# godk1122/IsaacLab

Hardware: AMD Instinct MI355X
Metric: env-steps/sec (whole node), Anymal-C rough 4096 envs/GPU, RSL-RL PPO iteration (collect+GAE+update) (higher is better)
Workload: dtype f32; 1 GPU; Isaac-Velocity-Rough-Anymal-C-v0, 4096 envs/GPU, T=24, 5 epochs x 4 minibatches, terrain 1204008 triangles, 4 state snapshots resident in HBM; parallelism=dp1, rollout=hipGraph, full_step=False, update=hipGraph (measured eager 16.72 ms, graph 16.06 ms), policy_params=571801

## Files before the change

isaaclab_amd/csrc/mlp_fwd.hip:

```cpp
#include "imx_internal.h"

typedef float f32x16 __attribute__((ext_vector_type(16)));

namespace {

constexpr int FW_KMAX = 256;
constexpr int FW_ROWS = 32;
constexpr int FW_KP = FW_KMAX + 4;
constexpr int FW_COLS = 128;

__device__ __forceinline__ int acc_row32(int reg, int half) { return (reg & 3) + 8 * (reg >> 2) + 4 * half; }

template <bool ELU, bool FULL>
__device__ __forceinline__ void store_rows(const f32x16& acc, float bias, float alpha, float* y, int64_t ldy, int rows, int half) {
#pragma unroll
    for (int g = 0; g < 4; ++g) {
        float* yg = y + (int64_t)(8 * g) * ldy;
#pragma unroll
        for (int j = 0; j < 4; ++j) {
            float x = acc[4 * g + j] + bias;
            if (ELU) {
                const float e = (__expf(fminf(x, 0.0f)) - 1.0f) * alpha;
                x = x <= 0.0f ? e : x;
            }
            if (FULL || 8 * g + j + 4 * half < rows) yg[0] = x;
            yg += ldy;
        }
    }
}

__device__ __forceinline__ void store_tile(const f32x16& acc, float bias, float alpha, int elu, float* y, int64_t ldy, int rows, int half) {
    if (rows >= FW_ROWS) {
        if (elu) store_rows<true, true>(acc, bias, alpha, y, ldy, rows, half);
        else store_rows<false, true>(acc, bias, alpha, y, ldy, rows, half);
    } else {
        if (elu) store_rows<true, false>(acc, bias, alpha, y, ldy, rows, half);
        else store_rows<false, false>(acc, bias, alpha, y, ldy, rows, half);
    }
}

struct FwArgs {
    int64_t M;
    int N, K;
    const float* X;
    int64_t ldx;
    const float* W;
    const float* b;
    float* Y;
    int64_t ldy;
    float alpha;
    int ncb;
    int rs;
    int64_t rps;
    int elu;
};

template <int NS, bool XVEC>
__global__ void __launch_bounds__(256, 2) k_mlp_fwd_elu(FwArgs a) {
    static_assert(NS % 4 == 0 && 2 * NS <= FW_KMAX, "step count");
    __shared__ __attribute__((aligned(16))) float sA[2][FW_ROWS * FW_KP];
    const int t = threadIdx.x, lane = t & 63, w = t >> 6, r = lane & 31, half = lane >> 5;
    const int cb = blockIdx.x % a.ncb, split = blockIdx.x / a.ncb;
    const int col = cb * FW_COLS + w * 32 + r;
    const bool col_ok = col < a.N;
    const int K = a.K;
    float breg[NS];
    {
        const float* wr = a.W + (size_t)(col_ok ? col : a.N - 1) * K;
#pragma unroll
        for (int s = 0; s < NS; ++s) {
            const int k = half * NS + s;
            const float v = wr[k < K ? k : K - 1];
            breg[s] = (k < K && col_ok) ? v : 0.0f;
        }
    }
    const float bias = col_ok ? a.b[col] : 0.0f;
    const int64_t m_begin = (int64_t)split * a.rps, m_end = min(m_begin + a.rps, a.M);
    const int ntile = (int)((m_end - m_begin + FW_ROWS - 1) / FW_ROWS);
    constexpr int C4 = 2 * NS / 4;
    constexpr int NV = (FW_ROWS * C4 + 255) / 256;
    float4 pre[NV];
    auto g_load = [&](int tile) {
        const int64_t row0 = m_begin + (int64_t)tile * FW_ROWS;
#pragma unroll
        for (int i = 0; i < NV; ++i) {
            const int idx = t + 256 * i;
            const int rr = idx / C4, c4 = idx - rr * C4;
            const int64_t row = min(row0 + rr, m_end - 1);
            const int k0 = 4 * c4;
            const float* p = a.X + row * a.ldx + (k0 < K ? k0 : 0);
            float4 v;
            if (XVEC) {
                v = *reinterpret_cast<const float4*>(p);
            } else {
                v.x = p[0];
                v.y = p[k0 + 1 < K ? 1 : 0];
                v.z = p[k0 + 2 < K ? 2 : 0];
                v.w = p[k0 + 3 < K ? 3 : 0];
            }
            v.x = k0 + 0 < K ? v.x : 0.f;
            v.y = k0 + 1 < K ? v.y : 0.f;
            v.z = k0 + 2 < K ? v.z : 0.f;
            v.w = k0 + 3 < K ? v.w : 0.f;
            pre[i] = v;
        }
    };
    auto s_store = [&](int buf) {
#pragma unroll
        for (int i = 0; i < NV; ++i) {
            const int idx = t + 256 * i;
            const int rr = idx / C4, c4 = idx - rr * C4;
            if (FW_ROWS * C4 % 256 == 0 || rr < FW_ROWS) *reinterpret_cast<float4*>(sA[buf] + rr * FW_KP + 4 * c4) = pre[i];
        }
    };
    if (ntile > 0) {
        g_load(0);
        s_store(0);
    }
    __syncthreads();
    for (int tile = 0; tile < ntile; ++tile) {
        const int buf = tile & 1;
        if (tile + 1 < ntile) g_load(tile + 1);
        f32x16 acc;
#pragma unroll
        for (int q = 0; q < 16; ++q) acc[q] = 0.0f;
        const float4* pa = reinterpret_cast<const float4*>(sA[buf] + r * FW_KP + half * NS);
#pragma unroll
        for (int s4 = 0; s4 < NS / 4; ++s4) {
            const float4 av = pa[s4];
            acc = __builtin_amdgcn_mfma_f32_32x32x2f32(av.x, breg[4 * s4 + 0], acc, 0, 0, 0);
            acc = __builtin_amdgcn_mfma_f32_32x32x2f32(av.y, breg[4 * s4 + 1], acc, 0, 0, 0);
            acc = __builtin_amdgcn_mfma_f32_32x32x2f32(av.z, breg[4 * s4 + 2], acc, 0, 0, 0);
            acc = __builtin_amdgcn_mfma_f32_32x32x2f32(av.w, breg[4 * s4 + 3], acc, 0, 0, 0);
        }
        const int64_t row0 = m_begin + (int64_t)tile * FW_ROWS;
        if (col_ok) store_tile(acc, bias, a.alpha, a.elu, a.Y + (row0 + 4 * half) * a.ldy + col, a.ldy, (int)min<int64_t>(m_end - row0, FW_ROWS), half);
        if (tile + 1 < ntile) s_store(buf ^ 1);
        __syncthreads();
    }
}

template <int NS>
__global__ void __launch_bounds__(256, 2) k_mlp_fwd_elu_dma(FwArgs a) {
    static_assert(NS % 4 == 0 && 2 * NS <= FW_KMAX, "step count");
    __shared__ __attribute__((aligned(16))) float sA[2][FW_ROWS * FW_KP];
    const int t = threadIdx.x, lane = t & 63, w = t >> 6, r = lane & 31, half = lane >> 5;
    const int nb = gridDim.x, per = nb >> 3;
    const int vb = (nb & 7) == 0 ? (int)(blockIdx.x & 7) * per + (int)(blockIdx.x >> 3) : (int)blockIdx.x;
    const int cb = vb % a.ncb, split = vb / a.ncb;
    const int col = cb * FW_COLS + w * 32 + r;
    const bool col_ok = col < a.N;
    const int K = a.K;
    float breg[NS];
    const unsigned lds_base = (unsigned)(uintptr_t)(__attribute__((address_space(3))) float*)&sA[0][0];
    {
        float* wl = &sA[0][0] + (w & 1) * (FW_ROWS * FW_KP);
        const int64_t blk0 = (int64_t)(cb * FW_COLS + w * 32) * K;
        const int64_t avail = min<int64_t>((int64_t)32 * K, (int64_t)a.N * K - blk0);
        const bool wvec = ((reinterpret_cast<uintptr_t>(a.W) & 15) == 0);
        const float* wrow = wl + r * K + half * NS;
        for (int turn = 0; turn < 2; ++turn) {
            if ((w >> 1) == turn) {
                const int64_t avail4 = avail & ~(int64_t)3;
                if (wvec && avail4 >= 4) {
                    const unsigned wl_lds = lds_base + (unsigned)((w & 1) * FW_ROWS * FW_KP * 4);
                    for (int i = 0; i < 32 * K; i += 256) {
                        const float* src = a.W + blk0 + min<int64_t>(i + 4 * lane, avail4 - 4);
                        unsigned keep;
                        asm volatile("s_mov_b32 %0, m0\n\ts_mov_b32 m0, %2\n\ts_nop 0\n\tglobal_load_lds_dwordx4 %1, off\n\ts_mov_b32 m0, %0"
                                     : "=&s"(keep) : "v"(src), "s"(__builtin_amdgcn_readfirstlane(wl_lds + (unsigned)i * 4u)) : "memory");
                    }
                    asm volatile("s_waitcnt vmcnt(0)" ::: "memory");
                    if (lane < avail - avail4) wl[avail4 + lane] = a.W[blk0 + avail4 + lane];
                } else {
                    for (int i = 4 * lane; i < 32 * K; i += 256) {
                        float4 v = make_float4(0.f, 0.f, 0.f, 0.f);
                        const float* src = a.W + blk0 + i;
                        if (i + 4 <= avail) {
                            if (wvec) v = *reinterpret_cast<const float4*>(src);
                            else { v.x = src[0]; v.y = src[1]; v.z = src[2]; v.w = src[3]; }
                        } else {
                            if (i + 0 < avail) v.x = src[0];
                            if (i + 1 < avail) v.y = src[1];
                            if (i + 2 < avail) v.z = src[2];
                        }
                        *reinterpret_cast<float4*>(wl + i) = v;
                    }
                }
#pragma unroll
                for (int s = 0; s < NS; ++s) {
                    const int k = half * NS + s;
                    const float v = wrow[k < K ? s : 0];
                    breg[s] = (k < K && col_ok) ? v : 0.0f;
                }
            }
            __syncthreads();
        }
    }
    const float bias = col_ok ? a.b[col] : 0.0f;
    const int64_t m_begin = (int64_t)split * a.rps, m_end = min(m_begin + a.rps, a.M);
    const int ntile = (int)((m_end - m_begin + FW_ROWS - 1) / FW_ROWS);
    constexpr int C4 = 2 * NS / 4;
    const int k0 = 4 * lane;
    const int64_t lane_off = (lane < C4 && k0 < K) ? k0 : 0;
    const int nz = 2 * NS - K;
    auto dma_tile = [&](int tile, int buf) {
        const int64_t row0 = m_begin + (int64_t)tile * FW_ROWS + 8 * w;
#pragma unroll
        for (int i = 0; i < 8; ++i) {
            const int64_t row = min(row0 + i, m_end - 1);
            const float* src = a.X + row * a.ldx + lane_off;
            const unsigned dst = lds_base + (unsigned)((buf * FW_ROWS + 8 * w + i) * FW_KP * 4);
            unsigned keep;
            asm volatile("s_mov_b32 %0, m0\n\ts_mov_b32 m0, %2\n\ts_nop 0\n\tglobal_load_lds_dwordx4 %1, off\n\ts_mov_b32 m0, %0"
                         : "=&s"(keep) : "v"(src), "s"(__builtin_amdgcn_readfirstlane(dst)) : "memory");
        }
    };
    const int zoff = lane < 8 * nz ? (8 * w + lane / nz) * FW_KP + K + lane % nz : -1;
    auto zero_tail = [&](int buf) {
        if (zoff >= 0) sA[buf][zoff] = 0.0f;
        for (int i = lane + 64; i < 8 * nz; i += 64) {
            const int rr = i / nz, c = i - rr * nz;
            sA[buf][(8 * w + rr) * FW_KP + K + c] = 0.0f;
        }
    };
    if (ntile > 0) {
        dma_tile(0, 0);
        asm volatile("s_waitcnt vmcnt(0)" ::: "memory");
        zero_tail(0);
    }
    __syncthreads();
    auto mfma_tile = [&](int buf, f32x16& acc) {
        const float4* pa = reinterpret_cast<const float4*>(sA[buf] + r * FW_KP + half * NS);
#pragma unroll
        for (int s4 = 0; s4 < NS / 4; ++s4) {
            const float4 av = pa[s4];
            acc = __builtin_amdgcn_mfma_f32_32x32x2f32(av.x, breg[4 * s4 + 0], acc, 0, 0, 0);
            acc = __builtin_amdgcn_mfma_f32_32x32x2f32(av.y, breg[4 * s4 + 1], acc, 0, 0, 0);
            acc = __builtin_amdgcn_mfma_f32_32x32x2f32(av.z, breg[4 * s4 + 2], acc, 0, 0, 0);
            acc = __builtin_amdgcn_mfma_f32_32x32x2f32(av.w, breg[4 * s4 + 3], acc, 0, 0, 0);
        }
    };
    auto end_of_tile = [&](int tile, bool stores_behind) {
        if (stores_behind) asm volatile("s_waitcnt vmcnt(16)" ::: "memory");
        else asm volatile("s_waitcnt vmcnt(0)" ::: "memory");
        if (tile + 1 < ntile) zero_tail((tile & 1) ^ 1);
        asm volatile("s_waitcnt lgkmcnt(0)" ::: "memory");
        __builtin_amdgcn_s_barrier();
    };
    const bool pipelined = a.elu && (cb + 1) * FW_COLS <= a.N && ntile >= 2;
    if (pipelined) {
        f32x16 prev;
#pragma unroll
        for (int q = 0; q < 16; ++q) prev[q] = 0.0f;
        dma_tile(1, 1);
        mfma_tile(0, prev);
        end_of_tile(0, false);
        for (int tile = 1; tile < ntile; ++tile) {
            const int buf = tile & 1;
            if (tile + 1 < ntile) dma_tile(tile + 1, buf ^ 1);
            f32x16 acc;
#pragma unroll
            for (int q = 0; q < 16; ++q) acc[q] = 0.0f;
            float* y = a.Y + (m_begin + (int64_t)(tile - 1) * FW_ROWS + 4 * half) * a.ldy + col;
            const float4* pa = reinterpret_cast<const float4*>(sA[buf] + r * FW_KP + half * NS);
            constexpr int EVERY = (NS / 4) / 16 >= 1 ? (NS / 4) / 16 : 1;
#pragma unroll
            for (int s4 = 0; s4 < NS / 4; ++s4) {
                const float4 av = pa[s4];
                acc = __builtin_amdgcn_mfma_f32_32x32x2f32(av.x, breg[4 * s4 + 0], acc, 0, 0, 0);
                acc = __builtin_amdgcn_mfma_f32_32x32x2f32(av.y, breg[4 * s4 + 1], acc, 0, 0, 0);
                acc = __builtin_amdgcn_mfma_f32_32x32x2f32(av.z, breg[4 * s4 + 2], acc, 0, 0, 0);
                acc = __builtin_amdgcn_mfma_f32_32x32x2f32(av.w, breg[4 * s4 + 3], acc, 0, 0, 0);
                if (s4 % EVERY == 0 && s4 / EVERY < 16) {
                    const int q = s4 / EVERY;
                    float x = prev[q] + bias;
                    const float e = (__expf(fminf(x, 0.0f)) - 1.0f) * a.alpha;
                    x = x <= 0.0f ? e : x;
                    *y = x;
                    y += ((q & 3) == 3 ? 5 : 1) * a.ldy;
                    __builtin_amdgcn_sched_barrier(0);
                }
            }
            static_assert(NS / 4 >= 16, "sixteen output rows need sixteen blocks");
            end_of_tile(tile, true);
            prev = acc;
        }
        const int64_t row0 = m_begin + (int64_t)(ntile - 1) * FW_ROWS;
        store_tile(prev, bias, a.alpha, a.elu, a.Y + (row0 + 4 * half) * a.ldy + col, a.ldy, (int)min<int64_t>(m_end - row0, FW_ROWS), half);
        return;
    }
    for (int tile = 0; tile < ntile; ++tile) {
        const int buf = tile & 1;
        if (tile + 1 < ntile) dma_tile(tile + 1, buf ^ 1);
        f32x16 acc;
#pragma unroll
        for (int q = 0; q < 16; ++q) acc[q] = 0.0f;
        mfma_tile(buf, acc);
        const int64_t row0 = m_begin + (int64_t)tile * FW_ROWS;
        asm volatile("s_waitcnt vmcnt(0)" ::: "memory");
        if (tile + 1 < ntile) zero_tail(buf ^ 1);
        if (col_ok) store_tile(acc, bias, a.alpha, a.elu, a.Y + (row0 + 4 * half) * a.ldy + col, a.ldy, (int)min<int64_t>(m_end - row0, FW_ROWS), half);
        asm volatile("s_waitcnt lgkmcnt(0)" ::: "memory");
        __builtin_amdgcn_s_barrier();
    }
}

template <bool XVEC>
void launch_fwd(const FwArgs& a, dim3 grid, hipStream_t st) {
    const dim3 block(256);
    const int ns = (a.K + 1) / 2;
    if (ns <= 32) hipLaunchKernelGGL((k_mlp_fwd_elu<32, XVEC>), grid, block, 0, st, a);
    else if (ns <= 64) hipLaunchKernelGGL((k_mlp_fwd_elu<64, XVEC>), grid, block, 0, st, a);
    else if (XVEC && ns <= 96) hipLaunchKernelGGL((k_mlp_fwd_elu_dma<96>), grid, block, 0, st, a);
    else if (XVEC && ns <= 120) hipLaunchKernelGGL((k_mlp_fwd_elu_dma<120>), grid, block, 0, st, a);
    else if (XVEC) hipLaunchKernelGGL((k_mlp_fwd_elu_dma<128>), grid, block, 0, st, a);
    else if (ns <= 96) hipLaunchKernelGGL((k_mlp_fwd_elu<96, false>), grid, block, 0, st, a);
    else if (ns <= 120) hipLaunchKernelGGL((k_mlp_fwd_elu<120, false>), grid, block, 0, st, a);
    else hipLaunchKernelGGL((k_mlp_fwd_elu<128, false>), grid, block, 0, st, a);
}

}

extern "C" int imx_mlp_fwd_elu(int64_t M, int N, int K, const float* X_d, int64_t ldx, const float* W_d, const float* b_d, float elu_alpha,
                               int apply_elu, float* Y_d, int64_t ldy, imx_stream_t stream) {
    IMX_REQUIRE(M > 0 && N > 0 && K > 0 && X_d && W_d && b_d && Y_d, "imx_mlp_fwd_elu: bad arguments");
    IMX_REQUIRE(K <= FW_KMAX, "imx_mlp_fwd_elu: %d in-features (at most %d: the weights of a column live in registers)", K, FW_KMAX);
    IMX_REQUIRE(ldx >= K && ldy >= N, "imx_mlp_fwd_elu: row pitch smaller than the row");
    static int num_cu = 0;
    if (num_cu == 0) {
        int dev = 0;
        if (hipGetDevice(&dev) != hipSuccess || hipDeviceGetAttribute(&num_cu, hipDeviceAttributeMultiprocessorCount, dev) != hipSuccess || num_cu <= 0)
            num_cu = 256;
    }
    FwArgs a;
    a.M = M; a.N = N; a.K = K; a.X = X_d; a.ldx = ldx; a.W = W_d; a.b = b_d; a.Y = Y_d; a.ldy = ldy; a.alpha = elu_alpha; a.elu = apply_elu;
    a.ncb = (N + FW_COLS - 1) / FW_COLS;
    int64_t rs = std::max<int64_t>(1, (2 * (int64_t)num_cu) / a.ncb);
    rs = std::min<int64_t>(rs, std::max<int64_t>(1, M / (4 * FW_ROWS)));
    a.rps = ((M + rs - 1) / rs + FW_ROWS - 1) / FW_ROWS * FW_ROWS;
    a.rs = (int)((M + a.rps - 1) / a.rps);
    const bool xvec = (ldx % 4 == 0) && ((reinterpret_cast<uintptr_t>(X_d) & 15) == 0) && (K % 4 == 0 || ldx >= ((K + 3) & ~3));
    const dim3 grid((unsigned)(a.ncb * a.rs));
    if (xvec) launch_fwd<true>(a, grid, (hipStream_t)stream);
    else launch_fwd<false>(a, grid, (hipStream_t)stream);
    IMX_HIP(hipGetLastError());
    return 0;
}
```

Before: 5.283 million env-steps/s.

## Split MLP forward into MFMA waves and helper waves for DMA and epilogue

Replaces the 256-thread DMA forward kernel for wide inputs (K>128) with a 512-thread warp-specialized kernel. Four waves run only MFMA and stage raw accumulators into LDS. Four helper waves prefetch X tiles with global_load_lds, then apply bias and ELU and write vectorized rows one tile behind. The weight block is loaded cooperatively by all waves in one pass, and the grid is sized for one workgroup per CU. This is meant to hide store and activation latency behind matrix math, at the cost of extra LDS traffic, lower occupancy and an extra barrier per tile.

```diff
diff --git a/isaaclab_amd/csrc/mlp_fwd.hip b/isaaclab_amd/csrc/mlp_fwd.hip
--- a/isaaclab_amd/csrc/mlp_fwd.hip
+++ b/isaaclab_amd/csrc/mlp_fwd.hip
@@ -1,6 +1,7 @@
 #include "imx_internal.h"
 
 typedef float f32x16 __attribute__((ext_vector_type(16)));
+typedef float f32x4 __attribute__((ext_vector_type(4)));
 
 namespace {
 
@@ -140,64 +141,36 @@
     }
 }
 
+constexpr int FW_SP = FW_COLS + 4;
+
 template <int NS>
-__global__ void __launch_bounds__(256, 2) k_mlp_fwd_elu_dma(FwArgs a) {
-    static_assert(NS % 4 == 0 && 2 * NS <= FW_KMAX, "step count");
-    __shared__ __attribute__((aligned(16))) float sA[2][FW_ROWS * FW_KP];
+struct FwLds {
+    static constexpr int TILE = FW_ROWS * FW_KP;
+    static constexpr int STAGE = FW_ROWS * FW_SP;
+    static constexpr int WBLK = FW_COLS * 2 * NS;
+    static constexpr bool T0_FREE = (TILE + WBLK) * 4 <= 160 * 1024;
+    static constexpr int W_OFF = T0_FREE ? TILE : 0;
+    static constexpr int LOOP = 2 * TILE + 2 * STAGE;
+    static constexpr int TOTAL = W_OFF + WBLK > LOOP ? W_OFF + WBLK : LOOP;
+};
+
+template <int NS>
+__global__ void __launch_bounds__(512, 1) k_mlp_fwd_elu_roles(FwArgs a) {
+    static_assert(NS % 8 == 0 && 2 * NS <= FW_KMAX, "step count");
+    using L = FwLds<NS>;
+    static_assert(L::TOTAL * 4 <= 160 * 1024, "LDS");
+    __shared__ __attribute__((aligned(16))) float lds[L::TOTAL];
+    float* const sA = lds;
+    float* const sS = lds + 2 * L::TILE;
+    float* const wl = lds + L::W_OFF;
     const int t = threadIdx.x, lane = t & 63, w = t >> 6, r = lane & 31, half = lane >> 5;
+    const bool helper = w >= 4;
+    const int h = w & 3;
     const int nb = gridDim.x, per = nb >> 3;
     const int vb = (nb & 7) == 0 ? (int)(blockIdx.x & 7) * per + (int)(blockIdx.x >> 3) : (int)blockIdx.x;
     const int cb = vb % a.ncb, split = vb / a.ncb;
-    const int col = cb * FW_COLS + w * 32 + r;
-    const bool col_ok = col < a.N;
     const int K = a.K;
-    float breg[NS];
-    const unsigned lds_base = (unsigned)(uintptr_t)(__attribute__((address_space(3))) float*)&sA[0][0];
-    {
-        float* wl = &sA[0][0] + (w & 1) * (FW_ROWS * FW_KP);
-        const int64_t blk0 = (int64_t)(cb * FW_COLS + w * 32) * K;
-        const int64_t avail = min<int64_t>((int64_t)32 * K, (int64_t)a.N * K - blk0);
-        const bool wvec = ((reinterpret_cast<uintptr_t>(a.W) & 15) == 0);
-        const float* wrow = wl + r * K + half * NS;
-        for (int turn = 0; turn < 2; ++turn) {
-            if ((w >> 1) == turn) {
-                const int64_t avail4 = avail & ~(int64_t)3;
-                if (wvec && avail4 >= 4) {
-                    const unsigned wl_lds = lds_base + (unsigned)((w & 1) * FW_ROWS * FW_KP * 4);
-                    for (int i = 0; i < 32 * K; i += 256) {
-                        const float* src = a.W + blk0 + min<int64_t>(i + 4 * lane, avail4 - 4);
-                        unsigned keep;
-                        asm volatile("s_mov_b32 %0, m0\n\ts_mov_b32 m0, %2\n\ts_nop 0\n\tglobal_load_lds_dwordx4 %1, off\n\ts_mov_b32 m0, %0"
-                                     : "=&s"(keep) : "v"(src), "s"(__builtin_amdgcn_readfirstlane(wl_lds + (unsigned)i * 4u)) : "memory");
-                    }
-                    asm volatile("s_waitcnt vmcnt(0)" ::: "memory");
-                    if (lane < avail - avail4) wl[avail4 + lane] = a.W[blk0 + avail4 + lane];
-                } else {
-                    for (int i = 4 * lane; i < 32 * K; i += 256) {
-                        float4 v = make_float4(0.f, 0.f, 0.f, 0.f);
-                        const float* src = a.W + blk0 + i;
-                        if (i + 4 <= avail) {
-                            if (wvec) v = *reinterpret_cast<const float4*>(src);
-                            else { v.x = src[0]; v.y = src[1]; v.z = src[2]; v.w = src[3]; }
-                        } else {
-                            if (i + 0 < avail) v.x = src[0];
-                            if (i + 1 < avail) v.y = src[1];
-                            if (i + 2 < avail) v.z = src[2];
-                        }
-                        *reinterpret_cast<float4*>(wl + i) = v;
-                    }
-                }
-#pragma unroll
-                for (int s = 0; s < NS; ++s) {
-                    const int k = half * NS + s;
-                    const float v = wrow[k < K ? s : 0];
-                    breg[s] = (k < K && col_ok) ? v : 0.0f;
-                }
-            }
-            __syncthreads();
-        }
-    }
-    const float bias = col_ok ? a.b[col] : 0.0f;
+    const unsigned lds_base = (unsigned)(uintptr_t)(__attribute__((address_space(3))) float*)&lds[0];
     const int64_t m_begin = (int64_t)split * a.rps, m_end = min(m_begin + a.rps, a.M);
     const int ntile = (int)((m_end - m_begin + FW_ROWS - 1) / FW_ROWS);
     constexpr int C4 = 2 * NS / 4;
@@ -205,116 +178,178 @@
     const int64_t lane_off = (lane < C4 && k0 < K) ? k0 : 0;
     const int nz = 2 * NS - K;
     auto dma_tile = [&](int tile, int buf) {
-        const int64_t row0 = m_begin + (int64_t)tile * FW_ROWS + 8 * w;
+        const int64_t row0 = m_begin + (int64_t)tile * FW_ROWS + 8 * h;
 #pragma unroll
         for (int i = 0; i < 8; ++i) {
             const int64_t row = min(row0 + i, m_end - 1);
             const float* src = a.X + row * a.ldx + lane_off;
-            const unsigned dst = lds_base + (unsigned)((buf * FW_ROWS + 8 * w + i) * FW_KP * 4);
+            const unsigned dst = lds_base + (unsigned)((buf * FW_ROWS + 8 * h + i) * FW_KP * 4);
             unsigned keep;
             asm volatile("s_mov_b32 %0, m0\n\ts_mov_b32 m0, %2\n\ts_nop 0\n\tglobal_load_lds_dwordx4 %1, off\n\ts_mov_b32 m0, %0"
                          : "=&s"(keep) : "v"(src), "s"(__builtin_amdgcn_readfirstlane(dst)) : "memory");
         }
     };
-    const int zoff = lane < 8 * nz ? (8 * w + lane / nz) * FW_KP + K + lane % nz : -1;
+    const int zoff = lane < 8 * nz ? (8 * h + lane / nz) * FW_KP + K + lane % nz : -1;
     auto zero_tail = [&](int buf) {
-        if (zoff >= 0) sA[buf][zoff] = 0.0f;
+        float* tb = sA + buf * L::TILE;
+        if (zoff >= 0) tb[zoff] = 0.0f;
         for (int i = lane + 64; i < 8 * nz; i += 64) {
             const int rr = i / nz, c = i - rr * nz;
-            sA[buf][(8 * w + rr) * FW_KP + K + c] = 0.0f;
-        }
-    };
-    if (ntile > 0) {
-        dma_tile(0, 0);
+            tb[(8 * h + rr) * FW_KP + K + c] = 0.0f;
+        }
+    };
+    {
+        const int64_t cb0 = (int64_t)cb * FW_COLS * K;
+        const int64_t avail = min<int64_t>((int64_t)FW_COLS * K, (int64_t)a.N * K - cb0);
+        const int64_t avail4 = avail & ~(int64_t)3;
+        const bool wdma = ((reinterpret_cast<uintptr_t>(a.W) & 15) == 0) && avail4 >= 4;
+        if (wdma) {
+            for (int i = 256 * w; i < FW_COLS * K; i += 8 * 256) {
+                const float* src = a.W + cb0 + min<int64_t>(i + 4 * lane, avail4 - 4);
+                unsigned keep;
+                asm volatile("s_mov_b32 %0, m0\n\ts_mov_b32 m0, %2\n\ts_nop 0\n\tglobal_load_lds_dwordx4 %1, off\n\ts_mov_b32 m0, %0"
+                             : "=&s"(keep) : "v"(src), "s"(__builtin_amdgcn_readfirstlane(lds_base + (unsigned)(L::W_OFF + i) * 4u)) : "memory");
+            }
+        } else {
+            for (int i = 4 * t; i < FW_COLS * K; i += 4 * 512) {
+                float4 v = make_float4(0.f, 0.f, 0.f, 0.f);
+                const float* src = a.W + cb0 + i;
+                if (i + 0 < avail) v.x = src[0];
+                if (i + 1 < avail) v.y = src[1];
+                if (i + 2 < avail) v.z = src[2];
+                if (i + 3 < avail) v.w = src[3];
+                *reinterpret_cast<float4*>(wl + i) = v;
+            }
+        }
+        if (L::T0_FREE && helper && ntile > 0) dma_tile(0, 0);
         asm volatile("s_waitcnt vmcnt(0)" ::: "memory");
-        zero_tail(0);
+        if (L::T0_FREE && helper && ntile > 0) zero_tail(0);
+        __syncthreads();
+        if (wdma && t < avail - avail4) wl[avail4 + t] = a.W[cb0 + avail4 + t];
+        __syncthreads();
+    }
+    if (!helper) {
+        const int col = cb * FW_COLS + w * 32 + r;
+        const bool col_ok = col < a.N;
+        float breg[NS];
+        {
+            const float* wrow = wl + (w * 32 + r) * K + half * NS;
+#pragma unroll
+            for (int s = 0; s < NS; ++s) {
+                const int k = half * NS + s;
+                const float v = wrow[k < K ? s : 0];
+                breg[s] = (k < K && col_ok) ? v : 0.0f;
+            }
+        }
+        asm volatile("s_waitcnt lgkmcnt(0)" ::: "memory");
+        if (!L::T0_FREE) __syncthreads();
+        __syncthreads();
+        for (int tile = 0; tile < ntile; ++tile) {
+            const int buf = tile & 1;
+            f32x16 acc;
+#pragma unroll
+            for (int q = 0; q < 16; ++q) acc[q] = 0.0f;
+            const float4* pa = reinterpret_cast<const float4*>(sA + buf * L::TILE + r * FW_KP + half * NS);
+            float4 op[2][2];
+            op[0][0] = pa[0];
+            op[0][1] = pa[1];
+#pragma unroll
+            for (int c = 0; c < NS / 8; ++c) {
+                if (c + 1 < NS / 8) {
+                    op[(c + 1) & 1][0] = pa[2 * c + 2];
+                    op[(c + 1) & 1][1] = pa[2 * c + 3];
+                }
+                __builtin_amdgcn_sched_barrier(0);
+#pragma unroll
+                for (int j = 0; j < 2; ++j) {
+                    const float4 av = op[c & 1][j];
+                    const int s = 8 * c + 4 * j;
+                    acc = __builtin_amdgcn_mfma_f32_32x32x2f32(breg[s + 0], av.x, acc, 0, 0, 0);
+                    acc = __builtin_amdgcn_mfma_f32_32x32x2f32(breg[s + 1], av.y, acc, 0, 0, 0);
+                    acc = __builtin_amdgcn_mfma_f32_32x32x2f32(breg[s + 2], av.z, acc, 0, 0, 0);
+                    acc = __builtin_amdgcn_mfma_f32_32x32x2f32(breg[s + 3], av.w, acc, 0, 0, 0);
+                }
+                __builtin_amdgcn_sched_barrier(0);
+            }
+            float* ps = sS + buf * L::STAGE + r * FW_SP + w * 32 + 4 * half;
+#pragma unroll
+            for (int g = 0; g < 4; ++g) *reinterpret_cast<float4*>(ps + 8 * g) = make_float4(acc[4 * g], acc[4 * g + 1], acc[4 * g + 2], acc[4 * g + 3]);
+            asm volatile("s_waitcnt lgkmcnt(0)" ::: "memory");
+            __builtin_amdgcn_s_barrier();
+        }
+        return;
+    }
+    const int c4 = lane & 31, rsub = lane >> 5;
+    const int colh = cb * FW_COLS + 4 * c4;
+    float4 b4;
+    b4.x = colh + 0 < a.N ? a.b[colh + 0] : 0.0f;
+    b4.y = colh + 1 < a.N ? a.b[colh + 1] : 0.0f;
+    b4.z = colh + 2 < a.N ? a.b[colh + 2] : 0.0f;
+    b4.w = colh + 3 < a.N ? a.b[colh + 3] : 0.0f;
+    const bool yvec = ((reinterpret_cast<uintptr_t>(a.Y) & 15) == 0) && (a.ldy & 3) == 0;
+    const bool wide = yvec && (cb + 1) * FW_COLS <= a.N;
+    const float alpha = a.alpha;
+    const int elu = a.elu;
+    auto act = [&](float x) {
+        const float e = (__expf(fminf(x, 0.0f)) - 1.0f) * alpha;
+        return x <= 0.0f ? e : x;
+    };
+    auto epilogue = [&](int tile, bool full) {
+        const int64_t row0 = m_begin + (int64_t)tile * FW_ROWS;
+        const int rows = full ? FW_ROWS : (int)min<int64_t>(m_end - row0, FW_ROWS);
+        const float* ps = sS + (tile & 1) * L::STAGE + (8 * h + rsub) * FW_SP + 4 * c4;
+        float* y = a.Y + (row0 + 8 * h + rsub) * a.ldy + colh;
+#pragma unroll
+        for (int i = 0; i < 4; ++i) {
+            float4 v = *reinterpret_cast<const float4*>(ps + 2 * i * FW_SP);
+            v.x += b4.x; v.y += b4.y; v.z += b4.z; v.w += b4.w;
+            if (elu) { v.x = act(v.x); v.y = act(v.y); v.z = act(v.z); v.w = act(v.w); }
+            float* yr = y + (int64_t)(2 * i) * a.ldy;
+            if (wide) {
+                if (full || 8 * h + rsub + 2 * i < rows) *reinterpret_cast<f32x4*>(yr) = f32x4{v.x, v.y, v.z, v.w};
+            } else if (8 * h + rsub + 2 * i < rows) {
+                if (colh + 0 < a.N) yr[0] = v.x;
+                if (colh + 1 < a.N) yr[1] = v.y;
+                if (colh + 2 < a.N) yr[2] = v.z;
+                if (colh + 3 < a.N) yr[3] = v.w;
+            }
+        }
+    };
+    if (!L::T0_FREE) {
+        __syncthreads();
+        if (ntile > 0) {
+            dma_tile(0, 0);
+            asm volatile("s_waitcnt vmcnt(0)" ::: "memory");
+            zero_tail(0);
+        }
     }
     __syncthreads();
-    auto mfma_tile = [&](int buf, f32x16& acc) {
-        const float4* pa = reinterpret_cast<const float4*>(sA[buf] + r * FW_KP + half * NS);
-#pragma unroll
-        for (int s4 = 0; s4 < NS / 4; ++s4) {
-            const float4 av = pa[s4];
-            acc = __builtin_amdgcn_mfma_f32_32x32x2f32(av.x, breg[4 * s4 + 0], acc, 0, 0, 0);
-            acc = __builtin_amdgcn_mfma_f32_32x32x2f32(av.y, breg[4 * s4 + 1], acc, 0, 0, 0);
-            acc = __builtin_amdgcn_mfma_f32_32x32x2f32(av.z, breg[4 * s4 + 2], acc, 0, 0, 0);
-            acc = __builtin_amdgcn_mfma_f32_32x32x2f32(av.w, breg[4 * s4 + 3], acc, 0, 0, 0);
-        }
-    };
-    auto end_of_tile = [&](int tile, bool stores_behind) {
-        if (stores_behind) asm volatile("s_waitcnt vmcnt(16)" ::: "memory");
+    for (int tile = 0; tile < ntile; ++tile) {
+        const bool more = tile + 1 < ntile;
+        if (more) dma_tile(tile + 1, (tile & 1) ^ 1);
+        if (tile > 0) epilogue(tile - 1, true);
+        if (tile > 0 && wide) asm volatile("s_waitcnt vmcnt(4)" ::: "memory");
         else asm volatile("s_waitcnt vmcnt(0)" ::: "memory");
-        if (tile + 1 < ntile) zero_tail((tile & 1) ^ 1);
+        if (more) zero_tail((tile & 1) ^ 1);
         asm volatile("s_waitcnt lgkmcnt(0)" ::: "memory");
         __builtin_amdgcn_s_barrier();
-    };
-    const bool pipelined = a.elu && (cb + 1) * FW_COLS <= a.N && ntile >= 2;
-    if (pipelined) {
-        f32x16 prev;
-#pragma unroll
-        for (int q = 0; q < 16; ++q) prev[q] = 0.0f;
-        dma_tile(1, 1);
-        mfma_tile(0, prev);
-        end_of_tile(0, false);
-        for (int tile = 1; tile < ntile; ++tile) {
-            const int buf = tile & 1;
-            if (tile + 1 < ntile) dma_tile(tile + 1, buf ^ 1);
-            f32x16 acc;
-#pragma unroll
-            for (int q = 0; q < 16; ++q) acc[q] = 0.0f;
-            float* y = a.Y + (m_begin + (int64_t)(tile - 1) * FW_ROWS + 4 * half) * a.ldy + col;
-            const float4* pa = reinterpret_cast<const float4*>(sA[buf] + r * FW_KP + half * NS);
-            constexpr int EVERY = (NS / 4) / 16 >= 1 ? (NS / 4) / 16 : 1;
-#pragma unroll
-            for (int s4 = 0; s4 < NS / 4; ++s4) {
-                const float4 av = pa[s4];
-                acc = __builtin_amdgcn_mfma_f32_32x32x2f32(av.x, breg[4 * s4 + 0], acc, 0, 0, 0);
-                acc = __builtin_amdgcn_mfma_f32_32x32x2f32(av.y, breg[4 * s4 + 1], acc, 0, 0, 0);
-                acc = __builtin_amdgcn_mfma_f32_32x32x2f32(av.z, breg[4 * s4 + 2], acc, 0, 0, 0);
-                acc = __builtin_amdgcn_mfma_f32_32x32x2f32(av.w, breg[4 * s4 + 3], acc, 0, 0, 0);
-                if (s4 % EVERY == 0 && s4 / EVERY < 16) {
-                    const int q = s4 / EVERY;
-                    float x = prev[q] + bias;
-                    const float e = (__expf(fminf(x, 0.0f)) - 1.0f) * a.alpha;
-                    x = x <= 0.0f ? e : x;
-                    *y = x;
-                    y += ((q & 3) == 3 ? 5 : 1) * a.ldy;
-                    __builtin_amdgcn_sched_barrier(0);
-                }
-            }
-            static_assert(NS / 4 >= 16, "sixteen output rows need sixteen blocks");
-            end_of_tile(tile, true);
-            prev = acc;
-        }
-        const int64_t row0 = m_begin + (int64_t)(ntile - 1) * FW_ROWS;
-        store_tile(prev, bias, a.alpha, a.elu, a.Y + (row0 + 4 * half) * a.ldy + col, a.ldy, (int)min<int64_t>(m_end - row0, FW_ROWS), half);
-        return;
-    }
-    for (int tile = 0; tile < ntile; ++tile) {
-        const int buf = tile & 1;
-        if (tile + 1 < ntile) dma_tile(tile + 1, buf ^ 1);
-        f32x16 acc;
-#pragma unroll
-        for (int q = 0; q < 16; ++q) acc[q] = 0.0f;
-        mfma_tile(buf, acc);
-        const int64_t row0 = m_begin + (int64_t)tile * FW_ROWS;
-        asm volatile("s_waitcnt vmcnt(0)" ::: "memory");
-        if (tile + 1 < ntile) zero_tail(buf ^ 1);
-        if (col_ok) store_tile(acc, bias, a.alpha, a.elu, a.Y + (row0 + 4 * half) * a.ldy + col, a.ldy, (int)min<int64_t>(m_end - row0, FW_ROWS), half);
-        asm volatile("s_waitcnt lgkmcnt(0)" ::: "memory");
-        __builtin_amdgcn_s_barrier();
-    }
+    }
+    if (ntile > 0) epilogue(ntile - 1, false);
 }
 
 template <bool XVEC>
 void launch_fwd(const FwArgs& a, dim3 grid, hipStream_t st) {
+    const int ns = (a.K + 1) / 2;
+    if (XVEC && ns > 64) {
+        const dim3 block(512);
+        if (ns <= 96) hipLaunchKernelGGL((k_mlp_fwd_elu_roles<96>), grid, block, 0, st, a);
+        else if (ns <= 120) hipLaunchKernelGGL((k_mlp_fwd_elu_roles<120>), grid, block, 0, st, a);
+        else hipLaunchKernelGGL((k_mlp_fwd_elu_roles<128>), grid, block, 0, st, a);
+        return;
+    }
     const dim3 block(256);
-    const int ns = (a.K + 1) / 2;
     if (ns <= 32) hipLaunchKernelGGL((k_mlp_fwd_elu<32, XVEC>), grid, block, 0, st, a);
     else if (ns <= 64) hipLaunchKernelGGL((k_mlp_fwd_elu<64, XVEC>), grid, block, 0, st, a);
-    else if (XVEC && ns <= 96) hipLaunchKernelGGL((k_mlp_fwd_elu_dma<96>), grid, block, 0, st, a);
-    else if (XVEC && ns <= 120) hipLaunchKernelGGL((k_mlp_fwd_elu_dma<120>), grid, block, 0, st, a);
-    else if (XVEC) hipLaunchKernelGGL((k_mlp_fwd_elu_dma<128>), grid, block, 0, st, a);
     else if (ns <= 96) hipLaunchKernelGGL((k_mlp_fwd_elu<96, false>), grid, block, 0, st, a);
     else if (ns <= 120) hipLaunchKernelGGL((k_mlp_fwd_elu<120, false>), grid, block, 0, st, a);
     else hipLaunchKernelGGL((k_mlp_fwd_elu<128, false>), grid, block, 0, st, a);
@@ -336,11 +371,12 @@
     FwArgs a;
     a.M = M; a.N = N; a.K = K; a.X = X_d; a.ldx = ldx; a.W = W_d; a.b = b_d; a.Y = Y_d; a.ldy = ldy; a.alpha = elu_alpha; a.elu = apply_elu;
     a.ncb = (N + FW_COLS - 1) / FW_COLS;
-    int64_t rs = std::max<int64_t>(1, (2 * (int64_t)num_cu) / a.ncb);
+    const bool xvec = (ldx % 4 == 0) && ((reinterpret_cast<uintptr_t>(X_d) & 15) == 0) && (K % 4 == 0 || ldx >= ((K + 3) & ~3));
+    const int wg_per_cu = (xvec && (K + 1) / 2 > 64) ? 1 : 2;
+    int64_t rs = std::max<int64_t>(1, (wg_per_cu * (int64_t)num_cu) / a.ncb);
     rs = std::min<int64_t>(rs, std::max<int64_t>(1, M / (4 * FW_ROWS)));
     a.rps = ((M + rs - 1) / rs + FW_ROWS - 1) / FW_ROWS * FW_ROWS;
     a.rs = (int)((M + a.rps - 1) / a.rps);
-    const bool xvec = (ldx % 4 == 0) && ((reinterpret_cast<uintptr_t>(X_d) & 15) == 0) && (K % 4 == 0 || ldx >= ((K + 3) & ~3));
     const dim3 grid((unsigned)(a.ncb * a.rs));
     if (xvec) launch_fwd<true>(a, grid, (hipStream_t)stream);
     else launch_fwd<false>(a, grid, (hipStream_t)stream);
```

Measured after the change: 5.343 million env-steps/s, median of 6. 1.1% higher.
